# visinf/style-seqcvae

Hardware: AMD Instinct MI355X
Metric: captions/sec (train step) (higher is better)
Workload: dtype f32; 1 GPU; C2 train step: fwd+bwd+allreduce+clip+SGD, B=64/GPU, R=36, F=2048, L=20 (T=21), Z=128, V=10000, E=1000, H=1200, A=768, SENTIMENT_VAE=1; global_batch=64, parallelism=dp1

## Files before the change

### include/ssc.h

```cpp
#ifndef SSC_H
#define SSC_H

#include <stddef.h>
#include <stdint.h>

#ifdef __cplusplus
extern "C" {
#endif

#define SSC_OK 0
#define SSC_EINVAL (-1)
#define SSC_EALIGN (-2)
#define SSC_EHIP (-3)
#define SSC_EWORKSPACE (-4)

#define SSC_MAX_SEG 6

int ssc_version(void);
int ssc_last_hip_error(void);
const char* ssc_arch(void);

typedef struct {
  const float* A; const float* B;
  int lda, ldb, K;
// ... 62 lines not shown
                     void* stream);

typedef struct {
  int B, H;
  const float* dh; int ld_dh;
  const float* dh2; int ld_dh2;
  const float* dc_in; int ld_dcin;
  const float* gates;
  const float* c_prev; int ld_cprev;
  const float* c_new; int ld_cnew;
  float* dG;
  float* dc_prev; int ld_dcprev;
  float* dgsum;
  const float* slabsA; int nA; size_t strideA;
  const float* slabsB; int nB; size_t strideB;
} ssc_lstm_bwd_desc;
int ssc_lstm_bwd(const ssc_lstm_bwd_desc* d, void* stream);
int ssc_lstm_bwd_x(const ssc_lstm_bwd_desc* d, const float* x, int ldx, const float* w, int ldw, int K, void* stream);

int ssc_attn_logits(const float* q, int ldq, const float* pv, const float* wa, int G, int R, int A, int rows_per_image,
                    float* logits, void* stream);
int ssc_attn_fwd(const float* q, int ldq, const float* pv, const float* wa, const float* mask, const float* feats,
                 int G, int R, int A, int F, int rows_per_image, float* logits, float* alpha, float* att, int ldatt,
                 void* stream);

int ssc_attn_weights(const float* q, int ldq, const float* pv, const float* wa, const float* mask, int G, int R, int A,
                     int rows_per_image, float* logits, float* alpha, void* stream);

int ssc_attn_pool(const float* alpha, const float* x, int G, int R, int D, int rows_per_image, float* out, int ldo,
                  void* stream);
int ssc_attn_fwd_pool(const float* q, int ldq, const float* pv, const float* wa, const float* mask, const float* feats,
                      int G, int R, int A, int F, int rows_per_image, float* logits, float* alpha, float* att, int ldatt,
                      const float* obj, int D, float* pool, int ldpool, void* stream);

int ssc_attn_bwd(const float* datt, int lddatt, const float* q, int ldq, const float* pv, const float* wa,
                 const float* alpha, const float* feats, int G, int R, int A, int F, float* dq, int lddq,
                 float* dpv_acc, float* dwa_acc, float* scratch_dalpha, void* stream);
int ssc_attn_bwd_pool(const float* datt, int lddatt, const float* q, int ldq, const float* pv, const float* wa,
                      const float* alpha, const float* feats, int G, int R, int A, int F, float* dq, int lddq,
                      float* dpv_acc, float* dwa_acc, float* scratch_dalpha, const float* obj, int D, const float* dpool_a,
                      int lddpa, int Da, const float* dpool_b, int lddpb, void* stream);

typedef struct {
  int B, Z;
  const float* mulv; int ldmulv; int nslab; size_t slab_stride;
  const float* bmu; const float* blv;
  const float* eps; int ldeps;
  int kld_mode;
  const float* sent; float pm_scale; float prior_var;
  const float* w;
  float* mu; float* lv; float* z; int ldz;
  float* kld_acc;
  const float* pm; int ldpm;
} ssc_latent_fwd_desc;
int ssc_latent_fwd(const ssc_latent_fwd_desc* d, void* stream);

// ... 289 lines not shown
```

### style-seqcvae_amd/csrc/attention.hip

```cpp
#include "ssc_common.h"

namespace {

constexpr int ATTN_RG = 8;
constexpr int ATTN_MAXA = 4096;
__global__ __launch_bounds__(256) void attn_logits_kernel(const float* __restrict__ q, int ldq, int nslab, size_t slab_stride,
                                                          float* __restrict__ q_out, int ldqo,
                                                          const float* __restrict__ pv, const float* __restrict__ wa,
                                                          int G, int R, int A, int rows_per_image,
                                                          float* __restrict__ logits, const int* __restrict__ rows,
                                                          const int* __restrict__ row_count) {
  __shared__ __attribute__((aligned(16))) float sq[ATTN_MAXA];
  const int groups = (R + ATTN_RG - 1) / ATTN_RG;
  int g = blockIdx.x / groups;
  const int grp = blockIdx.x - g * groups;
  if (rows) {
    if (g >= *row_count) return;
    g = rows[g];
  }
  const int tid = threadIdx.x, wave = tid >> 6, lane = tid & 63;
  const int img = g / rows_per_image;
  const float* qp = q + (size_t)g * ldq;
  const bool vec = ((A & 3) == 0) && ((ldq & 3) == 0) && ((ldqo & 3) == 0) && ((slab_stride & 3) == 0) && ssc_aligned16_dev(qp) &&
                   ssc_aligned16_dev(pv) && ssc_aligned16_dev(wa) && (!q_out || ssc_aligned16_dev(q_out));
// ... 199 lines not shown
      float4 b = *reinterpret_cast<const float4*>(fp + f);
      s += a.x * b.x + a.y * b.y + a.z * b.z + a.w * b.w;
    }
  } else {
    for (int f = lane; f < F; f += 64) s += dp[f] * fp[f];
  }
  if (obj) {
    const float* op = obj + (size_t)wid * D;
    for (int k = lane; k < D; k += 64)
      s += ((k < Da ? dpa[(size_t)g * lddpa + k] : 0.f) + (dpb ? dpb[(size_t)g * lddpb + k] : 0.f)) * op[k];
  }
  s = ssc_wave_sum(s);
  if (lane == 0) dalpha[wid] = s;
}

__global__ __launch_bounds__(256) void attn_bwd_apply_kernel(const float* __restrict__ q, int ldq,
                                                             const float* __restrict__ pv, const float* __restrict__ wa,
                                                             const float* __restrict__ alpha,
                                                             const float* __restrict__ dalpha, int G, int R, int A,
                                                             float* __restrict__ dq, int lddq, float* __restrict__ dpv_acc,
                                                             float* __restrict__ dwa_acc) {
  __shared__ float sdl[64 * MAXR_LANE];
  __shared__ float red[2][4][256];
  const int g = blockIdx.y, chunk = blockIdx.x, tid = threadIdx.x, lane = tid & 63, wave = tid >> 6;
  float c = 0.f;
  for (int r = lane; r < R; r += 64) c += alpha[(size_t)g * R + r] * dalpha[(size_t)g * R + r];
  c = ssc_wave_sum(c);
  if (wave == 0)
    for (int r = lane; r < R; r += 64) sdl[r] = alpha[(size_t)g * R + r] * (dalpha[(size_t)g * R + r] - c);
  __syncthreads();
  const int a0 = chunk * 256 + lane * 4;
  float dqa[4] = {0.f, 0.f, 0.f, 0.f}, dw[4] = {0.f, 0.f, 0.f, 0.f};
  const bool vec = ((A & 3) == 0) && ((ldq & 3) == 0) && ssc_aligned16_dev(q) && ssc_aligned16_dev(pv) &&
                   ssc_aligned16_dev(wa) && ssc_aligned16_dev(dpv_acc);
  if (vec) {
    if (a0 < A) {
      const float4 qv = *reinterpret_cast<const float4*>(q + (size_t)g * ldq + a0);
      const float4 wv = *reinterpret_cast<const float4*>(wa + a0);
      const float qa[4] = {qv.x, qv.y, qv.z, qv.w}, ww[4] = {wv.x, wv.y, wv.z, wv.w};
      for (int rb = wave; rb < R; rb += 4 * 5) {
        float4 p4[5], ac[5];
#pragma unroll
        for (int i = 0; i < 5; ++i) {
          const size_t off = ((size_t)g * R + min(rb + 4 * i, R - 1)) * A + a0;
// ... 146 lines not shown
  return ssc_attn_bwd_pool(datt, lddatt, q, ldq, pv, wa, alpha, feats, G, R, A, F, dq, lddq, dpv_acc, dwa_acc, scratch_dalpha,
                           nullptr, 0, nullptr, 0, 0, nullptr, 0, stream);
}

extern "C" int ssc_attn_bwd_pool(const float* datt, int lddatt, const float* q, int ldq, const float* pv, const float* wa,
                                 const float* alpha, const float* feats, int G, int R, int A, int F, float* dq, int lddq,
                                 float* dpv_acc, float* dwa_acc, float* scratch_dalpha, const float* obj, int D,
                                 const float* dpool_a, int lddpa, int Da, const float* dpool_b, int lddpb, void* stream) {
  if (!datt || !q || !pv || !wa || !alpha || !feats || !dq || !dpv_acc || !dwa_acc || !scratch_dalpha) return SSC_EINVAL;
  if (G <= 0 || R <= 0 || A <= 0 || F <= 0 || R > 64 * MAXR_LANE || lddatt < F || ldq < A || lddq < A) return SSC_EINVAL;
  if (obj && (!dpool_a || D <= 0 || Da < 0 || Da > D || lddpa < Da || (dpool_b && lddpb < D))) return SSC_EINVAL;
  SSC_LAUNCH(attn_dalpha_kernel, dim3(ssc_cdiv(G * R, 4)), dim3(256), 0, (hipStream_t)stream, datt, lddatt, feats,
                     G, R, F, scratch_dalpha, obj, D, dpool_a, lddpa, Da, dpool_b, lddpb);
  SSC_CHECK_LAUNCH();
  SSC_LAUNCH(attn_bwd_apply_kernel, dim3(ssc_cdiv(A, 256), G), dim3(256), 0, (hipStream_t)stream, q, ldq, pv, wa,
                     alpha, scratch_dalpha, G, R, A, dq, lddq, dpv_acc, dwa_acc);
  SSC_CHECK_LAUNCH();
  return SSC_OK;
}
```

### style-seqcvae_amd/csrc/pointwise.hip

```cpp
#include <type_traits>

#include <algorithm>

#include "ssc_common.h"

thread_local int ssc_tls_hip_error = 0;

extern "C" int ssc_version(void) { return 4; }
extern "C" int ssc_last_hip_error(void) { return ssc_tls_hip_error; }
extern "C" const char* ssc_arch(void) { return "gfx950"; }

namespace {

__global__ void feat_mask_kernel(const float* __restrict__ feats, int BR, int F, float* __restrict__ mask) {
  int row = blockIdx.x * (blockDim.x >> 6) + (threadIdx.x >> 6);
  int lane = threadIdx.x & 63;
  if (row >= BR) return;
  const float* p = feats + (size_t)row * F;
  float s = 0.f;
  for (int f = lane; f < F; f += 64) s += fabsf(p[f]);
  s = ssc_wave_sum(s);
  if (lane == 0) mask[row] = s > 0.f ? 1.f : 0.f;
}

// ... 623 lines not shown
      ssc_f32x4v acc = {0.f, 0.f, 0.f, 0.f};
      acc = __builtin_amdgcn_mfma_f32_16x16x4f32(av.x, bv.x, acc, 0, 0, 0);
      acc = __builtin_amdgcn_mfma_f32_16x16x4f32(av.y, bv.y, acc, 0, 0, 0);
      acc = __builtin_amdgcn_mfma_f32_16x16x4f32(av.z, bv.z, acc, 0, 0, 0);
      acc = __builtin_amdgcn_mfma_f32_16x16x4f32(av.w, bv.w, acc, 0, 0, 0);
      const int n = ct * 16 + r16;
#pragma unroll
      for (int i = 0; i < 4; ++i) {
        const int ob = b0 + rt * 16 + 4 * q4 + i;
        if (ob < d.B && n < NP) po[(size_t)ob * NP + n] = acc[i];
      }
    }
  }
}

__global__ void lstm_bwd_kernel(const ssc_lstm_bwd_desc d) {
  int j = blockIdx.x * blockDim.x + threadIdx.x;
  int b = blockIdx.y;
  if (j >= d.H) return;
  const int H = d.H, H4 = 4 * d.H;
  const float dcin = d.dc_in ? d.dc_in[(size_t)b * d.ld_dcin + j] : 0.f;
  const float* g = d.gates + (size_t)b * H4 + j;
  const float ig = g[0], fg = g[H], gg = g[2 * H], og = g[3 * H];
  const float cp = d.c_prev[(size_t)b * d.ld_cprev + j];
  const float cn = d.c_new[(size_t)b * d.ld_cnew + j];
  float dh = d.dh ? d.dh[(size_t)b * d.ld_dh + j] : 0.f;
  if (d.dh2) dh += d.dh2[(size_t)b * d.ld_dh2 + j];
  auto add_slabs = [&](const float* slabs, int n, size_t stride, auto uc) __attribute__((always_inline)) {
    constexpr int U = decltype(uc)::value;
    for (int s0 = 0; s0 < n; s0 += U) {
      float t[U];
#pragma unroll
      for (int u = 0; u < U; ++u) t[u] = slabs[(size_t)min(s0 + u, n - 1) * stride + (size_t)b * H + j];
#pragma unroll
      for (int u = 0; u < U; ++u) dh += (s0 + u < n) ? t[u] : 0.f;
    }
  };
  if (d.nA > 8) add_slabs(d.slabsA, d.nA, d.strideA, std::integral_constant<int, 16>{});
  else if (d.nA > 0) add_slabs(d.slabsA, d.nA, d.strideA, std::integral_constant<int, 8>{});
  if (d.nB > 8) add_slabs(d.slabsB, d.nB, d.strideB, std::integral_constant<int, 16>{});
  else if (d.nB > 0) add_slabs(d.slabsB, d.nB, d.strideB, std::integral_constant<int, 8>{});
// ... 40 lines not shown
      xr[u] = (k < K && xb < d.B) ? xp[k] : 0.f;
    }
    const int wj = j0 + (tid & 15);
#pragma unroll
    for (int u = 0; u < KMAX / 32; ++u) {
      const int k = (tid >> 4) + 32 * u;
      wr[u] = (k < K && wj < H) ? w[(size_t)k * ldw + wj] : 0.f;
    }
  }
  const float dcin = d.dc_in ? d.dc_in[(size_t)bc * d.ld_dcin + jc] : 0.f;
  const float* g = d.gates + (size_t)bc * H4 + jc;
  const float ig = g[0], fg = g[H], gg = g[2 * H], og = g[3 * H];
  const float cp = d.c_prev[(size_t)bc * d.ld_cprev + jc];
  const float cn = d.c_new[(size_t)bc * d.ld_cnew + jc];
  float dh = d.dh ? d.dh[(size_t)bc * d.ld_dh + jc] : 0.f;
  if (d.dh2) dh += d.dh2[(size_t)bc * d.ld_dh2 + jc];
  auto add_slabs = [&](const float* slabs, int n, size_t stride, auto uc) __attribute__((always_inline)) {
    constexpr int U = decltype(uc)::value;
    for (int s0 = 0; s0 < n; s0 += U) {
      float t[U];
#pragma unroll
      for (int u = 0; u < U; ++u) t[u] = slabs[(size_t)min(s0 + u, n - 1) * stride + (size_t)bc * H + jc];
#pragma unroll
      for (int u = 0; u < U; ++u) dh += (s0 + u < n) ? t[u] : 0.f;
    }
  };
  if (d.nA > 8) add_slabs(d.slabsA, d.nA, d.strideA, std::integral_constant<int, 16>{});
  else if (d.nA > 0) add_slabs(d.slabsA, d.nA, d.strideA, std::integral_constant<int, 8>{});
  if (d.nB > 8) add_slabs(d.slabsB, d.nB, d.strideB, std::integral_constant<int, 16>{});
  else if (d.nB > 0) add_slabs(d.slabsB, d.nB, d.strideB, std::integral_constant<int, 8>{});
// ... 530 lines not shown
  if (cpw < 1) cpw = 1;
  if (cpw > chunks) cpw = chunks;
  const size_t lds = ((size_t)R * 128 + 16 * (size_t)(R + 1)) * sizeof(float);
  if (lds > 64 * 1024) {
    if (hipFuncSetAttribute((const void*)lstm_fwd_img_kernel, hipFuncAttributeMaxDynamicSharedMemorySize, 80 * 1024) != hipSuccess) return SSC_EHIP;
  }
  SSC_LAUNCH(lstm_fwd_img_kernel, dim3(gx, nimg * ssc_cdiv(chunks, cpw)), dim3(512), lds, S(stream), *d, alpha, ldalpha, P, R,
             rows_per_image, cpw);
  SSC_CHECK_LAUNCH();
  return SSC_OK;
}

extern "C" int ssc_lstm_bwd(const ssc_lstm_bwd_desc* d, void* stream) {
  if (!d || d->B <= 0 || d->H <= 0 || !d->gates || !d->c_prev || !d->c_new || !d->dG || !d->dc_prev) return SSC_EINVAL;
  if ((d->nA > 0 && !d->slabsA) || (d->nB > 0 && !d->slabsB) || d->nA < 0 || d->nB < 0) return SSC_EINVAL;
  SSC_LAUNCH(lstm_bwd_kernel, dim3(ssc_cdiv(d->H, 128), d->B), dim3(128), 0, S(stream), *d);
  SSC_CHECK_LAUNCH();
  return SSC_OK;
}

extern "C" int ssc_lstm_fwd_p(const ssc_lstm_fwd_desc* d, const float* wp, int ldwp, int NP, float* pout, void* stream) {
  if (!d || d->B <= 0 || d->H <= 0 || !d->c_out || !d->h_out) return SSC_EINVAL;
  if (d->nslab < 0 || (d->nslab > 0 && !d->slabs)) return SSC_EINVAL;
  if (d->sent && !d->wcol) return SSC_EINVAL;
  if (d->add1 && d->rows_per_add1 <= 0) return SSC_EINVAL;
  if (!wp || !pout || NP <= 0 || NP > 256 || ldwp < d->H) return SSC_EINVAL;
  if (d->h_planes) return SSC_EINVAL;
  SSC_LAUNCH(lstm_fwd_p_kernel, dim3(ssc_cdiv(d->H, 16), ssc_cdiv(d->B, 32)), dim3(512), 0, S(stream), *d, wp, ldwp, NP, pout);
  SSC_CHECK_LAUNCH();
  return SSC_OK;
}

extern "C" int ssc_lstm_bwd_x(const ssc_lstm_bwd_desc* d, const float* x, int ldx, const float* w, int ldw, int K, void* stream) {
  if (!d || d->B <= 0 || d->H <= 0 || !d->gates || !d->c_prev || !d->c_new || !d->dG || !d->dc_prev) return SSC_EINVAL;
  if ((d->nA > 0 && !d->slabsA) || (d->nB > 0 && !d->slabsB) || d->nA < 0 || d->nB < 0) return SSC_EINVAL;
  if (!x || !w || K <= 0 || K > 768 || ldx < K || ldw < d->H) return SSC_EINVAL;
  const int KP = (K + 63) & ~63;
  const size_t lds = ((size_t)(32 + 16) * (KP + 4) + 4 * 32 * 17) * sizeof(float);
  const dim3 grid(ssc_cdiv(d->H, 16), ssc_cdiv(d->B, 32));
  if (K <= 256) {
    SSC_LAUNCH(lstm_bwd_x_kernel<256>, grid, dim3(512), lds, S(stream), *d, x, ldx, w, ldw, K);
  } else {
    if (hipFuncSetAttribute((const void*)lstm_bwd_x_kernel<768>, hipFuncAttributeMaxDynamicSharedMemorySize, 160 * 1024) != hipSuccess) return SSC_EHIP;
    if (lds > 160 * 1024) return SSC_EINVAL;
    SSC_LAUNCH(lstm_bwd_x_kernel<768>, grid, dim3(512), lds, S(stream), *d, x, ldx, w, ldw, K);
  }
  SSC_CHECK_LAUNCH();
  return SSC_OK;
}

// ... 179 lines not shown
```

### style-seqcvae_amd/csrc/sequence.hip

```cpp
#include <cstdlib>
#include <initializer_list>

#include "ssc_common.h"
#include "ssc_debug.h"

namespace {

inline size_t r4(size_t x) { return (x + 3) & ~(size_t)3; }

struct Layout {
  int B, R, L, T;
  int V, E, H, A, F, Z, S, tied;
  int Ep, Hp, Ap, Fp, Zp, Vp, H4, XW;
  int D, Dp, SC, NX;
  size_t wc_e, wc_d, pool, dpm;
  size_t total = 0;
  size_t act;
  size_t live;
  size_t tok, w, nvalid, sent_all, wcol_e, wcol_d, mask, avg, pv, emb, ga_static, ga_avg;
  size_t h1, c1, he, ce, hd, cd, gates_a, gates_e, gates_d, q, attn_logits, alpha, att, mu, lv, z, mulv;
  size_t slabs, slab_floats, logits, lse, proj;
  size_t sl_q, sl_mulv, sl_gh1, sl_ghd, sl_ghd2, sl_ghe, sl_dqw, sl_dhe, sl_dz, small_floats, wsum_att, wsum_dec, wz;
  size_t sl_ga, sl_ge, sl_gd, gate_floats;
  size_t dhdv, dga, dge, dgd, dga_sum, g_h1, g_c1, g_he, g_ce, g_cd, dz, dmulv, dx, dalpha, dq, dpv, dwa, demb, dproj;
// ... 57 lines not shown
  l.wsum_dec = l.take((size_t)l.H4 * l.Hp);
  l.wz = l.take((size_t)l.H4 * l.Zp);
  l.wc_e = l.take((size_t)l.H4 * l.Dp); l.wc_d = l.take((size_t)l.H4 * l.Dp);
  l.pool = l.take(TB * l.Dp); l.dpm = l.take((size_t)B * l.Dp);
  l.logits = l.take(TB * l.Vp);
  l.lse = l.take(2 * TB);
  l.proj = l.take(l.tied ? TB * l.Ep : 0);
  l.dhdv = l.take(TB * l.Hp);
  l.dga = l.take(TB * l.H4); l.dge = l.take(TB * l.H4); l.dgd = l.take(TB * l.H4);
  l.dga_sum = l.take((size_t)B * l.H4);
  l.g_h1 = l.take((size_t)B * l.Hp); l.g_c1 = l.take((size_t)B * l.Hp);
  l.g_he = l.take((size_t)B * l.Hp); l.g_ce = l.take((size_t)B * l.Hp);
  l.g_cd = l.take((size_t)B * l.Hp);
  l.dz = l.take((size_t)B * l.Zp);
  l.dmulv = l.take(TB * 2 * l.Z);
  l.dx = l.take((size_t)B * l.XW);
  l.dalpha = l.take((size_t)B * R);
  l.dq = l.take(TB * l.Ap);
  l.dpv = l.take((size_t)B * R * l.A);
  l.dwa = l.take((size_t)B * l.A);
  l.demb = l.take(TB * l.Ep);
  l.dproj = l.take(l.tied ? TB * l.Ep : 0);
  return l;
}

struct Seg {
  const float* A; int lda;
  const float* B; int ldb;
  int K;
};

struct Ctx {
// ... 497 lines not shown
  const int TB = T * B, XW = l.XW;
  int64_t* tok = (int64_t*)(W + l.tok);
  const size_t sH = (size_t)B * l.Hp;
  const float* hd_all = W + l.hd + sH;
  c.act_count = (const int*)(W + l.act); c.act_rows = c.act_count + 4;
  c.live_count = (const int*)(W + l.live); c.live_rows = c.live_count + 4;

  if (phases & (1u | 16u)) {
  SSC_TRY(ssc_ce_bwd(W + l.logits, l.Vp, tok + B, W + l.w, W + l.nvalid, W + l.lse, gl, T, B, V, st));
  const float* dlog = W + l.logits;
  {
    FillList f;
    f.add(W + l.dhdv, (size_t)TB * l.Hp);
    if (cfg->tied) f.add(W + l.dproj, (size_t)TB * l.Ep);
    for (size_t off : {l.g_c1, l.g_ce, l.g_cd}) f.add(W + off, sH);
    f.add(W + l.dx, (size_t)B * XW);
    f.add(W + l.dpv, (size_t)B * R * A);
    f.add(W + l.dwa, (size_t)B * A);
    f.add(W + l.dga_sum, (size_t)B * H4);
    SSC_TRY(fill_many(f, 0.f, st));
  }
  const int V4 = V >= 8 ? (V & ~3) : V;
  if (cfg->tied) {
    float* dP = W + l.dproj;
    SSC_TRY(gemm_rows(c, false, {{dlog, l.Vp, p->emb, p->ld_emb, V4}}, TB, E, dP, l.Ep));
    SSC_TRY(head_tail_rows(dlog, l.Vp, p->emb, p->ld_emb, V4, V, TB, E, dP, l.Ep, st));
    SSC_TRY(ssc_tanh_bwd(dP, l.Ep, W + l.proj, l.Ep, TB, E, st));
    SSC_TRY(gemm_rows(c, false, {{dP, l.Ep, p->proj_w, p->ld_proj_w, E}}, TB, H, W + l.dhdv, l.Hp));
    if (g->proj_w) SSC_TRY(gemm_dw(c, dP, l.Ep, hd_all, l.Hp, TB, E, H, g->proj_w, g->ld_proj_w));
    if (g->proj_b) SSC_TRY(ssc_colsum2(dP, l.Ep, TB, E, nullptr, g->proj_b, 1, nullptr, 0, c.slabs, st));
  } else {
    SSC_TRY(gemm_rows(c, false, {{dlog, l.Vp, p->out_w, p->ld_out_w, V4}}, TB, H, W + l.dhdv, l.Hp));
    SSC_TRY(head_tail_rows(dlog, l.Vp, p->out_w, p->ld_out_w, V4, V, TB, H, W + l.dhdv, l.Hp, st));
    if (g->out_w) {
      SSC_TRY(gemm_dw(c, dlog, l.Vp, hd_all, l.Hp, TB, V4, H, g->out_w, g->ld_out_w));
      SSC_TRY(head_tail_dw(dlog, l.Vp, hd_all, l.Hp, V4, V, TB, H, g->out_w, g->ld_out_w, st));
    }
    if (g->out_b) SSC_TRY(ssc_colsum2(dlog, l.Vp, TB, V, nullptr, g->out_b, 1, nullptr, 0, c.slabs, st));
  }
  }

  if (phases & (1u | 32u)) {
  float* dx = W + l.dx;
  int n_gh1 = 0, n_ghd = 0, n_ghd2 = 0, n_ghe = 0;
  const bool fc_adjacent_b = (p->fc_lv_w == p->fc_mean_w + (size_t)Z * p->ld_fc_mean_w) && p->ld_fc_lv_w == p->ld_fc_mean_w;
  const size_t sBH = (size_t)B * H;
  const int NX = l.NX;
  const size_t sBX = (size_t)B * NX;

  if (g_loop.on) { (void)hipEventRecord(g_loop.e[2], st); }
  for (int t = T - 1; t >= 0; --t) {
    float* dgd = W + l.dgd + (size_t)t * B * H4;
    float* dge = W + l.dge + (size_t)t * B * H4;
    float* dga = W + l.dga + (size_t)t * B * H4;
    float* dmulv = W + l.dmulv + (size_t)t * B * 2 * Z;
    float* dq = W + l.dq + (size_t)t * B * l.Ap;
    int ns = 0, n_dxd = 0, n_dxe = 0;
    {
      ssc_lstm_bwd_desc d{};
      d.B = B; d.H = H;
      d.dh = dx + F + H; d.ld_dh = XW;
      d.dh2 = W + l.dhdv + (size_t)t * B * l.Hp; d.ld_dh2 = l.Hp;
      d.slabsA = W + l.sl_ghd; d.nA = n_ghd; d.strideA = sBH;
      d.slabsB = W + l.sl_ghd2; d.nB = n_ghd2; d.strideB = sBH;
      d.dc_in = W + l.g_cd; d.ld_dcin = l.Hp;
      d.gates = W + l.gates_d + (size_t)t * B * H4;
      d.c_prev = W + l.cd + t * sH; d.ld_cprev = l.Hp;
      d.c_new = W + l.cd + (t + 1) * sH; d.ld_cnew = l.Hp;
      d.dG = dgd; d.dc_prev = W + l.g_cd; d.ld_dcprev = l.Hp;
      SSC_TRY(ssc_lstm_bwd(&d, st));
    }
    {
      ssc_gemm_desc d3[3];
      fill_desc(d3[0], true, false, {{dgd, H4, W + l.wz, l.Zp, H4}}, B, l.Zp);
      fill_desc(d3[1], true, false, {{dgd, H4, p->dec_w_ih, p->ld_dec_w_ih, H4}}, B, NX);
      fill_desc(d3[2], true, false, {{dgd, H4, p->dec_w_hh, p->ld_dec_w_hh, H4}}, B, H);
      const ssc_gemm_desc* dp[3] = {&d3[0], &d3[1], &d3[2]};
      float* regions[3] = {W + l.sl_dz, c.slabs, W + l.sl_ghd2};
      const size_t caps[3] = {l.small_floats, c.slab_floats / 2, l.small_floats};
      int ns3[3] = {0, 0, 0};
      SSC_TRY(ssc_gemm_slabs_group(dp, t > 0 ? 3 : 2, regions, caps, ns3, st));
      ns = ns3[0]; n_dxd = ns3[1]; n_ghd2 = ns3[2];
    }
    {
      ssc_latent_bwd_desc d{};
      d.B = B; d.Z = Z;
      d.dz = W + l.sl_dz; d.lddz = l.Zp; d.nslab = ns; d.slab_stride = (size_t)B * l.Zp;
      d.eps = bt->eps + (size_t)t * B * Z; d.ldeps = Z;
      d.mu = W + l.mu + (size_t)t * B * l.Zp; d.lv = W + l.lv + (size_t)t * B * l.Zp; d.ldz = l.Zp;
      d.kld_mode = cfg->kld_mode; d.sent = cfg->pm_scale != 0.f ? bt->sentiment : nullptr;
      d.pm_scale = cfg->pm_scale; d.prior_var = cfg->prior_var;
// ... 9 lines not shown
      d.dc_in = W + l.g_ce; d.ld_dcin = l.Hp;
      d.gates = W + l.gates_e + (size_t)t * B * H4;
      d.c_prev = W + l.ce + t * sH; d.ld_cprev = l.Hp;
      d.c_new = W + l.ce + (t + 1) * sH; d.ld_cnew = l.Hp;
      d.dG = dge; d.dc_prev = W + l.g_ce; d.ld_dcprev = l.Hp;
      if (fc_adjacent_b && 2 * Z <= 768) {
        SSC_TRY(ssc_lstm_bwd_x(&d, dmulv, 2 * Z, p->fc_mean_w, p->ld_fc_mean_w, 2 * Z, st));
      } else {
        SSC_TRY(gemm_to_slabs(c, W + l.sl_dhe, l.small_floats, true, false,
                              {{dmulv, 2 * Z, p->fc_mean_w, p->ld_fc_mean_w, Z}, {dmulv + Z, 2 * Z, p->fc_lv_w, p->ld_fc_lv_w, Z}}, B, H,
                              &ns));
        d.slabsB = W + l.sl_dhe; d.nB = ns; d.strideB = sBH;
        SSC_TRY(ssc_lstm_bwd(&d, st));
      }
    }
    {
      ssc_gemm_desc d2[2];
      fill_desc(d2[0], true, false, {{dge, H4, p->enc_w_ih, p->ld_enc_w_ih, H4}}, B, NX);
      fill_desc(d2[1], true, false, {{dge, H4, p->enc_w_hh, p->ld_enc_w_hh, H4}}, B, H);
      const ssc_gemm_desc* dp[2] = {&d2[0], &d2[1]};
      float* regions[2] = {c.slabs + (size_t)n_dxd * sBX, W + l.sl_ghe};
      const size_t caps[2] = {c.slab_floats - (size_t)n_dxd * sBX, l.small_floats};
      int ns2[2] = {0, 0};
      SSC_TRY(ssc_gemm_slabs_group(dp, t > 0 ? 2 : 1, regions, caps, ns2, st));
      n_dxe = ns2[0]; n_ghe = ns2[1];
    }
    SSC_TRY(ssc_reduce_slabs(c.slabs, n_dxd + n_dxe, sBX, B, NX, dx, XW, nullptr, 0, st));
    SSC_TRY(ssc_attn_bwd_pool(dx, XW, W + l.q + (size_t)t * B * l.Ap, l.Ap, W + l.pv, p->wa, W + l.alpha + (size_t)t * B * R,
                              bt->feats, B, R, A, F, dq, l.Ap, W + l.dpv, W + l.dwa, W + l.dalpha, l.D ? bt->obj_atts : nullptr, l.D,
                              dx + F + 2 * H, XW, l.SC, W + l.dpm, l.Dp, st));
    {
      ssc_lstm_bwd_desc d{};
      d.B = B; d.H = H;
      d.dh = dx + F; d.ld_dh = XW;
      d.slabsA = W + l.sl_gh1; d.nA = n_gh1; d.strideA = sBH;
      d.dc_in = W + l.g_c1; d.ld_dcin = l.Hp;
      d.gates = W + l.gates_a + (size_t)t * B * H4;
      d.c_prev = W + l.c1 + t * sH; d.ld_cprev = l.Hp;
      d.c_new = W + l.c1 + (t + 1) * sH; d.ld_cnew = l.Hp;
      d.dG = dga; d.dc_prev = W + l.g_c1; d.ld_dcprev = l.Hp;
      d.dgsum = W + l.dga_sum;
      const bool fused_q = A <= 768;
      if (fused_q) {
        SSC_TRY(ssc_lstm_bwd_x(&d, dq, l.Ap, p->wq, p->ld_wq, A, st));
      } else {
        SSC_TRY(gemm_to_slabs(c, W + l.sl_dqw, l.small_floats, true, false, {{dq, l.Ap, p->wq, p->ld_wq, A}}, B, H, &ns));
        d.slabsB = W + l.sl_dqw; d.nB = ns; d.strideB = sBH;
        SSC_TRY(ssc_lstm_bwd(&d, st));
      }
// ... 170 lines not shown
```

### style-seqcvae_amd/csrc/ssc_common.h

```cpp
#pragma once
#include <hip/hip_runtime.h>
#include <stddef.h>
#include <stdint.h>

#include "ssc.h"

extern thread_local int ssc_tls_hip_error;

#define SSC_LAUNCH(...)              \
  do {                               \
    (void)hipGetLastError();         \
    hipLaunchKernelGGL(__VA_ARGS__); \
  } while (0)

#define SSC_CHECK_LAUNCH()                         \
  do {                                             \
    hipError_t e__ = hipGetLastError();            \
    if (e__ != hipSuccess) {                       \
      ssc_tls_hip_error = (int)e__;                \
      return SSC_EHIP;                             \
    }                                              \
  } while (0)

#define SSC_TRY(expr)            \
// ... 10 lines not shown
  const char* e = getenv(name);
  return e ? atoi(e) : dflt;
}

static inline bool ssc_aligned16(const void* p) { return (((uintptr_t)p) & 15u) == 0; }
static inline int ssc_cdiv(int a, int b) { return (a + b - 1) / b; }
static inline size_t ssc_round_up(size_t a, size_t b) { return (a + b - 1) / b * b; }

#define SSC_WAVE 64
__device__ __forceinline__ bool ssc_aligned16_dev(const void* p) { return (((uintptr_t)p) & 15u) == 0; }

__device__ __forceinline__ float ssc_wave_sum(float v) {
#pragma unroll
  for (int o = 32; o > 0; o >>= 1) v += __shfl_xor(v, o, 64);
  return v;
}
__device__ __forceinline__ float ssc_wave_max(float v) {
#pragma unroll
  for (int o = 32; o > 0; o >>= 1) v = fmaxf(v, __shfl_xor(v, o, 64));
  return v;
}
__device__ __forceinline__ float ssc_sigmoid(float x) { return 1.0f / (1.0f + expf(-x)); }
__device__ __forceinline__ float ssc_tanh_fast(float x) {
  const float e = __builtin_amdgcn_exp2f(x * 2.8853900817779268f);
  return 1.0f - 2.0f * __builtin_amdgcn_rcpf(1.0f + e);
}

typedef float ssc_f32x4 __attribute__((ext_vector_type(4)));
typedef unsigned ssc_u32x2 __attribute__((ext_vector_type(2)));
typedef __fp16 ssc_h16x2 __attribute__((ext_vector_type(2)));
// ... 56 lines not shown
```

### style-seqcvae_amd/ssc_runtime/lib.py

```python
import ctypes as C
import os

_HERE = os.path.dirname(os.path.abspath(__file__))
DEBUG_ENV = os.environ.get("SSC_DEBUG", "") == "1"
LIB_PATH = (DEBUG_ENV and os.environ.get("SSC_LIB_PATH")) or os.path.join(os.path.dirname(_HERE), "libssc_hip.so")
SSC_MAX_SEG = 6

c_float_p = C.POINTER(C.c_float)
c_i64_p = C.POINTER(C.c_int64)
vp = C.c_void_p


class SscError(RuntimeError):
    CODES = {-1: "SSC_EINVAL", -2: "SSC_EALIGN", -3: "SSC_EHIP", -4: "SSC_EWORKSPACE"}

    def __init__(self, fn, rc, hip=0):
        super().__init__(f"{fn} failed: {self.CODES.get(rc, rc)}" + (f" (hipError {hip})" if rc == -3 else ""))
        self.rc = rc


class GemmSeg(C.Structure):
    _fields_ = [("A", vp), ("B", vp), ("lda", C.c_int), ("ldb", C.c_int), ("K", C.c_int),
                ("A16", vp), ("B16", vp), ("lda16", C.c_int), ("ldb16", C.c_int)]

# ... 8 lines not shown
class LstmFwdDesc(C.Structure):
    _fields_ = [("B", C.c_int), ("H", C.c_int), ("slabs", vp), ("nslab", C.c_int), ("slab_stride", C.c_size_t),
                ("add0", vp), ("ld_add0", C.c_int), ("add1", vp), ("ld_add1", C.c_int), ("rows_per_add1", C.c_int),
                ("b_ih", vp), ("b_hh", vp), ("sent", vp), ("wcol", vp), ("ldwcol", C.c_int), ("c_prev", vp),
                ("ld_cprev", C.c_int), ("gates_out", vp), ("c_out", vp), ("ld_cout", C.c_int), ("h_out", vp),
                ("ld_hout", C.c_int), ("add0_rows", vp), ("slab_rows", vp), ("slabs2", vp), ("nslab2", C.c_int),
                ("slab2_stride", C.c_size_t), ("slab2_rows", vp), ("c_prev_rows", vp), ("rows", vp), ("row_count", vp),
                ("h_planes", vp), ("ld_hplanes", C.c_int), ("planes_scale", vp)]


class LstmBwdDesc(C.Structure):
    _fields_ = [("B", C.c_int), ("H", C.c_int), ("dh", vp), ("ld_dh", C.c_int), ("dh2", vp), ("ld_dh2", C.c_int),
                ("dc_in", vp), ("ld_dcin", C.c_int), ("gates", vp), ("c_prev", vp), ("ld_cprev", C.c_int),
                ("c_new", vp), ("ld_cnew", C.c_int), ("dG", vp), ("dc_prev", vp), ("ld_dcprev", C.c_int), ("dgsum", vp),
                ("slabsA", vp), ("nA", C.c_int), ("strideA", C.c_size_t), ("slabsB", vp), ("nB", C.c_int),
                ("strideB", C.c_size_t)]


class LatentFwdDesc(C.Structure):
    _fields_ = [("B", C.c_int), ("Z", C.c_int), ("mulv", vp), ("ldmulv", C.c_int), ("nslab", C.c_int),
                ("slab_stride", C.c_size_t), ("bmu", vp), ("blv", vp), ("eps", vp), ("ldeps", C.c_int),
                ("kld_mode", C.c_int), ("sent", vp), ("pm_scale", C.c_float), ("prior_var", C.c_float), ("w", vp),
                ("mu", vp), ("lv", vp), ("z", vp), ("ldz", C.c_int), ("kld_acc", vp), ("pm", vp), ("ldpm", C.c_int)]


class LatentBwdDesc(C.Structure):
    _fields_ = [("B", C.c_int), ("Z", C.c_int), ("dz", vp), ("lddz", C.c_int), ("eps", vp), ("ldeps", C.c_int),
                ("mu", vp), ("lv", vp), ("ldz", C.c_int), ("kld_mode", C.c_int), ("sent", vp), ("pm_scale", C.c_float),
                ("prior_var", C.c_float), ("w", vp), ("gk", vp), ("dmulv", vp), ("lddmulv", C.c_int),
                ("nslab", C.c_int), ("slab_stride", C.c_size_t), ("pm", vp), ("ldpm", C.c_int), ("dpm", vp), ("lddpm", C.c_int)]

# ... 98 lines not shown
    "ssc_prep_tokens": (_i, [vp, _i, _i, _i, _i, vp, vp, vp, vp]),
    "ssc_embed_gather": (_i, [vp, _i, vp, _i, _i, vp, _i, vp]),
    "ssc_embed_scatter_add": (_i, [vp, _i, vp, _i, _i, vp, _i, _i, vp]),
    "ssc_lstm_fwd": (_i, [C.POINTER(LstmFwdDesc), vp]),
    "ssc_lstm_fwd_z": (_i, [C.POINTER(LstmFwdDesc), vp, _i, vp, _i, _i, vp]),
    "ssc_lstm_fwd_p": (_i, [C.POINTER(LstmFwdDesc), vp, _i, _i, vp, vp]),
    "ssc_lstm_fwd_img": (_i, [C.POINTER(LstmFwdDesc), vp, _i, vp, _i, _i, vp]),
    "ssc_lstm_bwd_x": (_i, [C.POINTER(LstmBwdDesc), vp, _i, vp, _i, _i, vp]),
    "ssc_lstm_bwd": (_i, [C.POINTER(LstmBwdDesc), vp]),
    "ssc_attn_logits": (_i, [vp, _i, vp, vp, _i, _i, _i, _i, vp, vp]),
    "ssc_attn_fwd": (_i, [vp, _i, vp, vp, vp, vp, _i, _i, _i, _i, _i, vp, vp, vp, _i, vp]),
    "ssc_attn_weights": (_i, [vp, _i, vp, vp, vp, _i, _i, _i, _i, vp, vp, vp]),
    "ssc_attn_pool": (_i, [vp, vp, _i, _i, _i, _i, vp, _i, vp]),
    "ssc_attn_fwd_pool": (_i, [vp, _i, vp, vp, vp, vp, _i, _i, _i, _i, _i, vp, vp, vp, _i, vp, _i, vp, _i, vp]),
    "ssc_attn_bwd_pool": (_i, [vp, _i, vp, _i, vp, vp, vp, vp, _i, _i, _i, _i, vp, _i, vp, vp, vp, vp, _i, vp, _i, _i, vp, _i, vp]),
    "ssc_attn_bwd": (_i, [vp, _i, vp, _i, vp, vp, vp, vp, _i, _i, _i, _i, vp, _i, vp, vp, vp, vp]),
    "ssc_latent_fwd": (_i, [C.POINTER(LatentFwdDesc), vp]),
    "ssc_latent_prior_sample": (_i, [vp, _i, vp, _f, _f, _i, _i, vp, _i, vp]),
    "ssc_latent_prior_sample_pm": (_i, [vp, _i, vp, _i, vp, _i, vp, _f, _f, _i, _i, vp, _i, vp]),
    "ssc_latent_bwd": (_i, [C.POINTER(LatentBwdDesc), vp]),
    "ssc_ce_fwd": (_i, [vp, _i, vp, vp, vp, _i, _i, _i, vp, vp, vp]),
    "ssc_ce_bwd": (_i, [vp, _i, vp, vp, vp, vp, vp, _i, _i, _i, vp]),
    "ssc_log_softmax": (_i, [vp, _i, _i, _i, vp, _i, vp]),
    "ssc_colsum": (_i, [vp, _i, _i, _i, vp, vp, _i, _i, vp]),
    "ssc_colsum2": (_i, [vp, _i, _i, _i, vp, vp, _i, vp, _i, vp, vp]),
    "ssc_copy_strided": (_i, [vp, _sz, _i, vp, vp]),
    "ssc_bias_tanh": (_i, [vp, _i, _i, _i, vp, vp]),
    "ssc_tanh_bwd": (_i, [vp, _i, vp, _i, _i, _i, vp]),
    "ssc_fill": (_i, [vp, _sz, _f, vp]),
    "ssc_sq_norm": (_i, [vp, _sz, vp, vp, vp]),
# ... 111 lines not shown
```

Baseline: 7590 captions/s.

## Consume dx GEMM slabs directly in attention and LSTM backward, skip slab reduction

When there are no object features (D==0), the backward loop no longer reduces the decoder and encoder dx GEMM slabs into a dense dx buffer. A new attention dalpha kernel sums the slabs on the fly and splits the F dimension across four blocks, writing partial dalpha values that the apply kernel adds together. The LSTM backward kernels gain two extra strided slab lists so they read dh straight from the slabs, including the previous step's encoder slabs. The decoder input GEMM also narrows to F+H columns and uses a summed hidden weight. This removes a reduce pass and the dx round-trip per timestep, at the cost of repeated slab reads and more complex indexing.

```diff
diff --git a/include/ssc.h b/include/ssc.h
--- a/include/ssc.h
+++ b/include/ssc.h
@@ -100,6 +100,8 @@
   float* dgsum;
   const float* slabsA; int nA; size_t strideA;
   const float* slabsB; int nB; size_t strideB;
+  const float* slabsC; int nC; size_t strideC; int ldC;
+  const float* slabsD; int nD; size_t strideD; int ldD;
 } ssc_lstm_bwd_desc;
 int ssc_lstm_bwd(const ssc_lstm_bwd_desc* d, void* stream);
 int ssc_lstm_bwd_x(const ssc_lstm_bwd_desc* d, const float* x, int ldx, const float* w, int ldw, int K, void* stream);
@@ -126,6 +128,11 @@
                       const float* alpha, const float* feats, int G, int R, int A, int F, float* dq, int lddq,
                       float* dpv_acc, float* dwa_acc, float* scratch_dalpha, const float* obj, int D, const float* dpool_a,
                       int lddpa, int Da, const float* dpool_b, int lddpb, void* stream);
+
+int ssc_attn_bwd_slabs(const float* datt_a, int na, size_t stride_a, int lda, const float* datt_b, int nb, size_t stride_b, int ldb,
+                       const float* q, int ldq, const float* pv, const float* wa, const float* alpha, const float* feats, int G,
+                       int R, int A, int F, float* dq, int lddq, float* dpv_acc, float* dwa_acc, float* scratch_dalpha,
+                       void* stream);
 
 typedef struct {
   int B, Z;
diff --git a/style-seqcvae_amd/csrc/attention.hip b/style-seqcvae_amd/csrc/attention.hip
--- a/style-seqcvae_amd/csrc/attention.hip
+++ b/style-seqcvae_amd/csrc/attention.hip
@@ -237,20 +237,75 @@
   if (lane == 0) dalpha[wid] = s;
 }
 
+constexpr int ATTN_DALPHA_PARTS = 4;
+__global__ __launch_bounds__(256) void attn_dalpha_slabs_kernel(const float* __restrict__ sa, int na, size_t stride_a, int lda,
+                                                                const float* __restrict__ sb, int nb, size_t stride_b, int ldb,
+                                                                const float* __restrict__ feats, int G, int R, int F, int CW,
+                                                                float* __restrict__ part) {
+  extern __shared__ __attribute__((aligned(16))) float sdatt[];
+  const int g = blockIdx.y, p = blockIdx.x, tid = threadIdx.x, lane = tid & 63, wave = tid >> 6;
+  const int c0 = p * CW;
+  const int cw = max(0, min(CW, F - c0));
+  for (int f = tid; f < cw; f += 256) {
+    float v = 0.f;
+    if (na > 8) v += ssc_slab_sum<16>(sa, na, stride_a, (size_t)g * lda + c0 + f);
+    else if (na > 0) v += ssc_slab_sum<8>(sa, na, stride_a, (size_t)g * lda + c0 + f);
+    if (nb > 8) v += ssc_slab_sum<16>(sb, nb, stride_b, (size_t)g * ldb + c0 + f);
+    else if (nb > 0) v += ssc_slab_sum<8>(sb, nb, stride_b, (size_t)g * ldb + c0 + f);
+    sdatt[f] = v;
+  }
+  __syncthreads();
+  const float* fg = feats + (size_t)g * R * F + c0;
+  const bool vec = ((F & 3) == 0) && ssc_aligned16_dev(feats);
+  for (int rb = wave; rb < R; rb += 12) {
+    float s[3] = {0.f, 0.f, 0.f};
+    const float* fp[3];
+#pragma unroll
+    for (int i = 0; i < 3; ++i) fp[i] = fg + (size_t)min(rb + 4 * i, R - 1) * F;
+    if (vec) {
+      for (int f = lane * 4; f < cw; f += 256) {
+        float4 b4[3];
+#pragma unroll
+        for (int i = 0; i < 3; ++i) b4[i] = *reinterpret_cast<const float4*>(fp[i] + f);
+        const float4 a4 = *reinterpret_cast<const float4*>(sdatt + f);
+#pragma unroll
+        for (int i = 0; i < 3; ++i) s[i] += a4.x * b4[i].x + a4.y * b4[i].y + a4.z * b4[i].z + a4.w * b4[i].w;
+      }
+    } else {
+      for (int f = lane; f < cw; f += 64) {
+        const float a1 = sdatt[f];
+#pragma unroll
+        for (int i = 0; i < 3; ++i) s[i] += a1 * fp[i][f];
+      }
+    }
+#pragma unroll
+    for (int i = 0; i < 3; ++i) {
+      const float t = ssc_wave_sum(s[i]);
+      const int r = rb + 4 * i;
+      if (lane == 0 && r < R) part[((size_t)p * G + g) * R + r] = t;
+    }
+  }
+}
+
 __global__ __launch_bounds__(256) void attn_bwd_apply_kernel(const float* __restrict__ q, int ldq,
                                                              const float* __restrict__ pv, const float* __restrict__ wa,
                                                              const float* __restrict__ alpha,
-                                                             const float* __restrict__ dalpha, int G, int R, int A,
+                                                             const float* __restrict__ dalpha, int nparts, int G, int R, int A,
                                                              float* __restrict__ dq, int lddq, float* __restrict__ dpv_acc,
                                                              float* __restrict__ dwa_acc) {
   __shared__ float sdl[64 * MAXR_LANE];
   __shared__ float red[2][4][256];
   const int g = blockIdx.y, chunk = blockIdx.x, tid = threadIdx.x, lane = tid & 63, wave = tid >> 6;
+  auto dal = [&](int r) -> float {
+    float v = dalpha[(size_t)g * R + r];
+    for (int p = 1; p < nparts; ++p) v += dalpha[((size_t)p * G + g) * R + r];
+    return v;
+  };
   float c = 0.f;
-  for (int r = lane; r < R; r += 64) c += alpha[(size_t)g * R + r] * dalpha[(size_t)g * R + r];
+  for (int r = lane; r < R; r += 64) c += alpha[(size_t)g * R + r] * dal(r);
   c = ssc_wave_sum(c);
   if (wave == 0)
-    for (int r = lane; r < R; r += 64) sdl[r] = alpha[(size_t)g * R + r] * (dalpha[(size_t)g * R + r] - c);
+    for (int r = lane; r < R; r += 64) sdl[r] = alpha[(size_t)g * R + r] * (dal(r) - c);
   __syncthreads();
   const int a0 = chunk * 256 + lane * 4;
   float dqa[4] = {0.f, 0.f, 0.f, 0.f}, dw[4] = {0.f, 0.f, 0.f, 0.f};
@@ -427,7 +482,25 @@
                      G, R, F, scratch_dalpha, obj, D, dpool_a, lddpa, Da, dpool_b, lddpb);
   SSC_CHECK_LAUNCH();
   SSC_LAUNCH(attn_bwd_apply_kernel, dim3(ssc_cdiv(A, 256), G), dim3(256), 0, (hipStream_t)stream, q, ldq, pv, wa,
-                     alpha, scratch_dalpha, G, R, A, dq, lddq, dpv_acc, dwa_acc);
-  SSC_CHECK_LAUNCH();
-  return SSC_OK;
-}
+                     alpha, scratch_dalpha, 1, G, R, A, dq, lddq, dpv_acc, dwa_acc);
+  SSC_CHECK_LAUNCH();
+  return SSC_OK;
+}
+
+extern "C" int ssc_attn_bwd_slabs(const float* datt_a, int na, size_t stride_a, int lda, const float* datt_b, int nb, size_t stride_b,
+                                  int ldb, const float* q, int ldq, const float* pv, const float* wa, const float* alpha,
+                                  const float* feats, int G, int R, int A, int F, float* dq, int lddq, float* dpv_acc,
+                                  float* dwa_acc, float* scratch_dalpha, void* stream) {
+  if (!q || !pv || !wa || !alpha || !feats || !dq || !dpv_acc || !dwa_acc || !scratch_dalpha) return SSC_EINVAL;
+  if (G <= 0 || R <= 0 || A <= 0 || F <= 0 || R > 64 * MAXR_LANE || ldq < A || lddq < A) return SSC_EINVAL;
+  if (na < 0 || nb < 0 || na + nb < 1 || (na > 0 && (!datt_a || lda < F)) || (nb > 0 && (!datt_b || ldb < F))) return SSC_EINVAL;
+  const int CW = (ssc_cdiv(F, ATTN_DALPHA_PARTS) + 3) & ~3;
+  if ((size_t)CW * sizeof(float) > 64 * 1024) return SSC_EINVAL;
+  SSC_LAUNCH(attn_dalpha_slabs_kernel, dim3(ATTN_DALPHA_PARTS, G), dim3(256), (size_t)CW * sizeof(float), (hipStream_t)stream,
+             datt_a, na, stride_a, lda, datt_b, nb, stride_b, ldb, feats, G, R, F, CW, scratch_dalpha);
+  SSC_CHECK_LAUNCH();
+  SSC_LAUNCH(attn_bwd_apply_kernel, dim3(ssc_cdiv(A, 256), G), dim3(256), 0, (hipStream_t)stream, q, ldq, pv, wa, alpha,
+             scratch_dalpha, ATTN_DALPHA_PARTS, G, R, A, dq, lddq, dpv_acc, dwa_acc);
+  SSC_CHECK_LAUNCH();
+  return SSC_OK;
+}
diff --git a/style-seqcvae_amd/csrc/pointwise.hip b/style-seqcvae_amd/csrc/pointwise.hip
--- a/style-seqcvae_amd/csrc/pointwise.hip
+++ b/style-seqcvae_amd/csrc/pointwise.hip
@@ -661,6 +661,14 @@
   }
 }
 
+__device__ __forceinline__ float lstm_bwd_strided_lists(const ssc_lstm_bwd_desc& d, int b, int j, float dh) {
+  if (d.nC > 8) dh += ssc_slab_sum<16>(d.slabsC, d.nC, d.strideC, (size_t)b * d.ldC + j);
+  else if (d.nC > 0) dh += ssc_slab_sum<8>(d.slabsC, d.nC, d.strideC, (size_t)b * d.ldC + j);
+  if (d.nD > 8) dh += ssc_slab_sum<16>(d.slabsD, d.nD, d.strideD, (size_t)b * d.ldD + j);
+  else if (d.nD > 0) dh += ssc_slab_sum<8>(d.slabsD, d.nD, d.strideD, (size_t)b * d.ldD + j);
+  return dh;
+}
+
 __global__ void lstm_bwd_kernel(const ssc_lstm_bwd_desc d) {
   int j = blockIdx.x * blockDim.x + threadIdx.x;
   int b = blockIdx.y;
@@ -672,6 +680,7 @@
   const float cp = d.c_prev[(size_t)b * d.ld_cprev + j];
   const float cn = d.c_new[(size_t)b * d.ld_cnew + j];
   float dh = d.dh ? d.dh[(size_t)b * d.ld_dh + j] : 0.f;
+  dh = lstm_bwd_strided_lists(d, b, j, dh);
   if (d.dh2) dh += d.dh2[(size_t)b * d.ld_dh2 + j];
   auto add_slabs = [&](const float* slabs, int n, size_t stride, auto uc) __attribute__((always_inline)) {
     constexpr int U = decltype(uc)::value;
@@ -742,6 +751,7 @@
   const float cp = d.c_prev[(size_t)bc * d.ld_cprev + jc];
   const float cn = d.c_new[(size_t)bc * d.ld_cnew + jc];
   float dh = d.dh ? d.dh[(size_t)bc * d.ld_dh + jc] : 0.f;
+  dh = lstm_bwd_strided_lists(d, bc, jc, dh);
   if (d.dh2) dh += d.dh2[(size_t)bc * d.ld_dh2 + jc];
   auto add_slabs = [&](const float* slabs, int n, size_t stride, auto uc) __attribute__((always_inline)) {
     constexpr int U = decltype(uc)::value;
@@ -1302,6 +1312,7 @@
 extern "C" int ssc_lstm_bwd(const ssc_lstm_bwd_desc* d, void* stream) {
   if (!d || d->B <= 0 || d->H <= 0 || !d->gates || !d->c_prev || !d->c_new || !d->dG || !d->dc_prev) return SSC_EINVAL;
   if ((d->nA > 0 && !d->slabsA) || (d->nB > 0 && !d->slabsB) || d->nA < 0 || d->nB < 0) return SSC_EINVAL;
+  if (d->nC < 0 || d->nD < 0 || (d->nC > 0 && (!d->slabsC || d->ldC < d->H)) || (d->nD > 0 && (!d->slabsD || d->ldD < d->H))) return SSC_EINVAL;
   SSC_LAUNCH(lstm_bwd_kernel, dim3(ssc_cdiv(d->H, 128), d->B), dim3(128), 0, S(stream), *d);
   SSC_CHECK_LAUNCH();
   return SSC_OK;
@@ -1322,6 +1333,7 @@
 extern "C" int ssc_lstm_bwd_x(const ssc_lstm_bwd_desc* d, const float* x, int ldx, const float* w, int ldw, int K, void* stream) {
   if (!d || d->B <= 0 || d->H <= 0 || !d->gates || !d->c_prev || !d->c_new || !d->dG || !d->dc_prev) return SSC_EINVAL;
   if ((d->nA > 0 && !d->slabsA) || (d->nB > 0 && !d->slabsB) || d->nA < 0 || d->nB < 0) return SSC_EINVAL;
+  if (d->nC < 0 || d->nD < 0 || (d->nC > 0 && (!d->slabsC || d->ldC < d->H)) || (d->nD > 0 && (!d->slabsD || d->ldD < d->H))) return SSC_EINVAL;
   if (!x || !w || K <= 0 || K > 768 || ldx < K || ldw < d->H) return SSC_EINVAL;
   const int KP = (K + 63) & ~63;
   const size_t lds = ((size_t)(32 + 16) * (KP + 4) + 4 * 32 * 17) * sizeof(float);
diff --git a/style-seqcvae_amd/csrc/sequence.hip b/style-seqcvae_amd/csrc/sequence.hip
--- a/style-seqcvae_amd/csrc/sequence.hip
+++ b/style-seqcvae_amd/csrc/sequence.hip
@@ -95,8 +95,8 @@
   l.g_cd = l.take((size_t)B * l.Hp);
   l.dz = l.take((size_t)B * l.Zp);
   l.dmulv = l.take(TB * 2 * l.Z);
-  l.dx = l.take((size_t)B * l.XW);
-  l.dalpha = l.take((size_t)B * R);
+  l.dx = l.take(l.D ? (size_t)B * l.XW : 0);
+  l.dalpha = l.take((size_t)4 * B * R);
   l.dq = l.take(TB * l.Ap);
   l.dpv = l.take((size_t)B * R * l.A);
   l.dwa = l.take((size_t)B * l.A);
@@ -624,7 +624,7 @@
     f.add(W + l.dhdv, (size_t)TB * l.Hp);
     if (cfg->tied) f.add(W + l.dproj, (size_t)TB * l.Ep);
     for (size_t off : {l.g_c1, l.g_ce, l.g_cd}) f.add(W + off, sH);
-    f.add(W + l.dx, (size_t)B * XW);
+    if (l.D) f.add(W + l.dx, (size_t)B * XW);
     f.add(W + l.dpv, (size_t)B * R * A);
     f.add(W + l.dwa, (size_t)B * A);
     f.add(W + l.dga_sum, (size_t)B * H4);
@@ -651,12 +651,17 @@
   }
 
   if (phases & (1u | 32u)) {
+  const bool slab_dx = l.D == 0;
   float* dx = W + l.dx;
   int n_gh1 = 0, n_ghd = 0, n_ghd2 = 0, n_ghe = 0;
   const bool fc_adjacent_b = (p->fc_lv_w == p->fc_mean_w + (size_t)Z * p->ld_fc_mean_w) && p->ld_fc_lv_w == p->ld_fc_mean_w;
   const size_t sBH = (size_t)B * H;
   const int NX = l.NX;
   const size_t sBX = (size_t)B * NX;
+  const int ND = slab_dx ? F + H : NX;
+  const size_t sBD = (size_t)B * ND;
+  const float* dxe_prev = nullptr;
+  int n_dxe_prev = 0;
 
   if (g_loop.on) { (void)hipEventRecord(g_loop.e[2], st); }
   for (int t = T - 1; t >= 0; --t) {
@@ -669,7 +674,8 @@
     {
       ssc_lstm_bwd_desc d{};
       d.B = B; d.H = H;
-      d.dh = dx + F + H; d.ld_dh = XW;
+      if (!slab_dx) { d.dh = dx + F + H; d.ld_dh = XW; }
+      else if (n_dxe_prev > 0) { d.slabsC = dxe_prev + F + H; d.nC = n_dxe_prev; d.strideC = sBX; d.ldC = NX; }
       d.dh2 = W + l.dhdv + (size_t)t * B * l.Hp; d.ld_dh2 = l.Hp;
       d.slabsA = W + l.sl_ghd; d.nA = n_ghd; d.strideA = sBH;
       d.slabsB = W + l.sl_ghd2; d.nB = n_ghd2; d.strideB = sBH;
@@ -683,8 +689,9 @@
     {
       ssc_gemm_desc d3[3];
       fill_desc(d3[0], true, false, {{dgd, H4, W + l.wz, l.Zp, H4}}, B, l.Zp);
-      fill_desc(d3[1], true, false, {{dgd, H4, p->dec_w_ih, p->ld_dec_w_ih, H4}}, B, NX);
-      fill_desc(d3[2], true, false, {{dgd, H4, p->dec_w_hh, p->ld_dec_w_hh, H4}}, B, H);
+      fill_desc(d3[1], true, false, {{dgd, H4, p->dec_w_ih, p->ld_dec_w_ih, H4}}, B, ND);
+      if (slab_dx) fill_desc(d3[2], true, false, {{dgd, H4, W + l.wsum_dec, l.Hp, H4}}, B, H);
+      else fill_desc(d3[2], true, false, {{dgd, H4, p->dec_w_hh, p->ld_dec_w_hh, H4}}, B, H);
       const ssc_gemm_desc* dp[3] = {&d3[0], &d3[1], &d3[2]};
       float* regions[3] = {W + l.sl_dz, c.slabs, W + l.sl_ghd2};
       const size_t caps[3] = {l.small_floats, c.slab_floats / 2, l.small_floats};
@@ -724,25 +731,38 @@
         SSC_TRY(ssc_lstm_bwd(&d, st));
       }
     }
+    const size_t dxe_off = slab_dx ? r4((size_t)n_dxd * sBD) : (size_t)n_dxd * sBX;
+    float* dxe = c.slabs + dxe_off;
     {
       ssc_gemm_desc d2[2];
       fill_desc(d2[0], true, false, {{dge, H4, p->enc_w_ih, p->ld_enc_w_ih, H4}}, B, NX);
       fill_desc(d2[1], true, false, {{dge, H4, p->enc_w_hh, p->ld_enc_w_hh, H4}}, B, H);
       const ssc_gemm_desc* dp[2] = {&d2[0], &d2[1]};
-      float* regions[2] = {c.slabs + (size_t)n_dxd * sBX, W + l.sl_ghe};
-      const size_t caps[2] = {c.slab_floats - (size_t)n_dxd * sBX, l.small_floats};
+      float* regions[2] = {dxe, W + l.sl_ghe};
+      const size_t caps[2] = {c.slab_floats - dxe_off, l.small_floats};
       int ns2[2] = {0, 0};
       SSC_TRY(ssc_gemm_slabs_group(dp, t > 0 ? 2 : 1, regions, caps, ns2, st));
       n_dxe = ns2[0]; n_ghe = ns2[1];
     }
-    SSC_TRY(ssc_reduce_slabs(c.slabs, n_dxd + n_dxe, sBX, B, NX, dx, XW, nullptr, 0, st));
-    SSC_TRY(ssc_attn_bwd_pool(dx, XW, W + l.q + (size_t)t * B * l.Ap, l.Ap, W + l.pv, p->wa, W + l.alpha + (size_t)t * B * R,
-                              bt->feats, B, R, A, F, dq, l.Ap, W + l.dpv, W + l.dwa, W + l.dalpha, l.D ? bt->obj_atts : nullptr, l.D,
-                              dx + F + 2 * H, XW, l.SC, W + l.dpm, l.Dp, st));
+    dxe_prev = dxe; n_dxe_prev = n_dxe;
+    if (slab_dx) {
+      SSC_TRY(ssc_attn_bwd_slabs(c.slabs, n_dxd, sBD, ND, dxe, n_dxe, sBX, NX, W + l.q + (size_t)t * B * l.Ap, l.Ap, W + l.pv, p->wa,
+                                 W + l.alpha + (size_t)t * B * R, bt->feats, B, R, A, F, dq, l.Ap, W + l.dpv, W + l.dwa, W + l.dalpha, st));
+    } else {
+      SSC_TRY(ssc_reduce_slabs(c.slabs, n_dxd + n_dxe, sBX, B, NX, dx, XW, nullptr, 0, st));
+      SSC_TRY(ssc_attn_bwd_pool(dx, XW, W + l.q + (size_t)t * B * l.Ap, l.Ap, W + l.pv, p->wa, W + l.alpha + (size_t)t * B * R,
+                                bt->feats, B, R, A, F, dq, l.Ap, W + l.dpv, W + l.dwa, W + l.dalpha, bt->obj_atts, l.D,
+                                dx + F + 2 * H, XW, l.SC, W + l.dpm, l.Dp, st));
+    }
     {
       ssc_lstm_bwd_desc d{};
       d.B = B; d.H = H;
-      d.dh = dx + F; d.ld_dh = XW;
+      if (slab_dx) {
+        d.slabsC = c.slabs + F; d.nC = n_dxd; d.strideC = sBD; d.ldC = ND;
+        d.slabsD = dxe + F; d.nD = n_dxe; d.strideD = sBX; d.ldD = NX;
+      } else {
+        d.dh = dx + F; d.ld_dh = XW;
+      }
       d.slabsA = W + l.sl_gh1; d.nA = n_gh1; d.strideA = sBH;
       d.dc_in = W + l.g_c1; d.ld_dcin = l.Hp;
       d.gates = W + l.gates_a + (size_t)t * B * H4;
diff --git a/style-seqcvae_amd/csrc/ssc_common.h b/style-seqcvae_amd/csrc/ssc_common.h
--- a/style-seqcvae_amd/csrc/ssc_common.h
+++ b/style-seqcvae_amd/csrc/ssc_common.h
@@ -48,6 +48,18 @@
 #pragma unroll
   for (int o = 32; o > 0; o >>= 1) v += __shfl_xor(v, o, 64);
   return v;
+}
+template <int U>
+__device__ __forceinline__ float ssc_slab_sum(const float* __restrict__ slabs, int n, size_t stride, size_t off) {
+  float acc = 0.f;
+  for (int s0 = 0; s0 < n; s0 += U) {
+    float t[U];
+#pragma unroll
+    for (int u = 0; u < U; ++u) t[u] = slabs[(size_t)min(s0 + u, n - 1) * stride + off];
+#pragma unroll
+    for (int u = 0; u < U; ++u) acc += (s0 + u < n) ? t[u] : 0.f;
+  }
+  return acc;
 }
 __device__ __forceinline__ float ssc_wave_max(float v) {
 #pragma unroll
diff --git a/style-seqcvae_amd/ssc_runtime/lib.py b/style-seqcvae_amd/ssc_runtime/lib.py
--- a/style-seqcvae_amd/ssc_runtime/lib.py
+++ b/style-seqcvae_amd/ssc_runtime/lib.py
@@ -46,7 +46,8 @@
                 ("dc_in", vp), ("ld_dcin", C.c_int), ("gates", vp), ("c_prev", vp), ("ld_cprev", C.c_int),
                 ("c_new", vp), ("ld_cnew", C.c_int), ("dG", vp), ("dc_prev", vp), ("ld_dcprev", C.c_int), ("dgsum", vp),
                 ("slabsA", vp), ("nA", C.c_int), ("strideA", C.c_size_t), ("slabsB", vp), ("nB", C.c_int),
-                ("strideB", C.c_size_t)]
+                ("strideB", C.c_size_t), ("slabsC", vp), ("nC", C.c_int), ("strideC", C.c_size_t), ("ldC", C.c_int),
+                ("slabsD", vp), ("nD", C.c_int), ("strideD", C.c_size_t), ("ldD", C.c_int)]
 
 
 class LatentFwdDesc(C.Structure):
@@ -175,6 +176,8 @@
     "ssc_attn_pool": (_i, [vp, vp, _i, _i, _i, _i, vp, _i, vp]),
     "ssc_attn_fwd_pool": (_i, [vp, _i, vp, vp, vp, vp, _i, _i, _i, _i, _i, vp, vp, vp, _i, vp, _i, vp, _i, vp]),
     "ssc_attn_bwd_pool": (_i, [vp, _i, vp, _i, vp, vp, vp, vp, _i, _i, _i, _i, vp, _i, vp, vp, vp, vp, _i, vp, _i, _i, vp, _i, vp]),
+    "ssc_attn_bwd_slabs": (_i, [vp, _i, _sz, _i, vp, _i, _sz, _i, vp, _i, vp, vp, vp, vp, _i, _i, _i, _i, vp, _i, vp, vp,
+                                vp, vp]),
     "ssc_attn_bwd": (_i, [vp, _i, vp, _i, vp, vp, vp, vp, _i, _i, _i, _i, vp, _i, vp, vp, vp, vp]),
     "ssc_latent_fwd": (_i, [C.POINTER(LatentFwdDesc), vp]),
     "ssc_latent_prior_sample": (_i, [vp, _i, vp, _f, _f, _i, _i, vp, _i, vp]),
```

New measurement: 7605 captions/s, median of 4. Within noise of the previous version (+0.2%).
